# ayotoasset/AdditiveCausalExpansion

Measured on AMD Instinct MI355X. Metric: log-marg-lik+grad evals/sec at n=16384,d=20; Cholesky GF/s vs MFMA peak, higher is better.
Workload: dtype f64; 1 GPU; C2: n=16384, d=20, Matern32, ns basis B=10, fp64; one para_update (kernel assembly + SPD inverse/log-det + all P gradients + RMSE/evidence + Nadam step) per step; n=16384, p=20, B=10, kernel=Matern32, parallelism=single

## Files before the change

additivecausalexpansion_amd/__init__.py:

```python
from ._lib import AceError, Context, default_context, lib
from .native import (
    DMat, Adam_cpp, Nadam_cpp, Nesterov_cpp, coef_contract, grad_Matern_cpp, grad_SE_cpp,
    invkernel_cpp, kernmat_Matern32_cpp, kernmat_Matern32_symmetric_cpp, kernmat_SE_cpp,
    kernmat_SE_symmetric_cpp, mu_solution_cpp, ncs_basis, ncs_basis_deriv, norm_clip_cpp,
    normalize_test, normalize_train, pred_cpp, pred_marginal_cpp, robust_levels, stats_cpp)
from .model import (
    DeviceModel, KernelClass_Matern32_R6, KernelClass_SE_R6, comm_unique_id, optAdam, optNadam,
    optNesterov, set_optimizer)
from .r6 import R6KernelMatern32, R6KernelSE
from .train import (
    AceFit, ace_train, coef_posterior, linear_spline, ns_spline, predict_ace, response_surface,
    robust_treatment, set_basis, set_initial_parameters, square_spline)
```

additivecausalexpansion_amd/_lib.py:

```python
from __future__ import annotations

import ctypes
import os
import threading

import numpy as np

_HERE = os.path.dirname(os.path.abspath(__file__))
LIB_PATH = os.environ.get("ACE_LIB_PATH") or os.path.join(_HERE, "libace_hip.so")

ACE_KERNEL_SE = 0
ACE_KERNEL_MATERN32 = 1
KIND = {"SE": ACE_KERNEL_SE, "Matern32": ACE_KERNEL_MATERN32}

_D = ctypes.POINTER(ctypes.c_double)
_I64 = ctypes.c_int64
_I32 = ctypes.POINTER(ctypes.c_int32)
_vp = ctypes.c_void_p

SIGNATURES = {
    "ace_abi_version": (ctypes.c_int, []),
    "ace_create": (ctypes.c_int, [ctypes.c_int, ctypes.POINTER(_vp)]),
    "ace_destroy": (None, [_vp]),
    "ace_last_error": (ctypes.c_char_p, [_vp]),
# ... 35 lines not shown
                                    _vp, _vp, ctypes.c_double, ctypes.c_double, _D, _D, _D]),
    "ace_pred_marginal_dev": (ctypes.c_int, [_vp, _I64, _I64, _D, _D, ctypes.c_double,
                                             ctypes.c_double, _vp, _vp, _vp, ctypes.c_double,
                                             ctypes.c_double, ctypes.c_double, ctypes.c_int, _D,
                                             _D, _D, _D]),
    "ace_nesterov": (ctypes.c_int, [_I64, ctypes.c_double, ctypes.c_double, _D, _D, _D]),
    "ace_nadam": (ctypes.c_int, [_I64, ctypes.c_double, ctypes.c_double, ctypes.c_double,
                                 ctypes.c_double, ctypes.c_double, _D, _D, _D, _D]),
    "ace_adam": (ctypes.c_int, [_I64, ctypes.c_double, ctypes.c_double, ctypes.c_double,
                                ctypes.c_double, ctypes.c_double, _D, _D, _D, _D]),
    "ace_norm_clip": (None, [ctypes.c_int, _I64, _D, ctypes.c_double]),
    "ace_ncs_basis": (ctypes.c_int, [_I64, _D, _I64, _D, _D, ctypes.POINTER(_I64)]),
    "ace_ncs_basis_deriv": (ctypes.c_int, [_I64, _D, _I64, _D, _D, ctypes.POINTER(_I64)]),
    "ace_normalize_train": (ctypes.c_int, [_I64, ctypes.c_int, ctypes.c_int, _D, _D, _D, _D]),
    "ace_normalize_test": (ctypes.c_int, [_I64, ctypes.c_int, ctypes.c_int, _D, _D, _D, _I64]),
    "ace_model_create": (ctypes.c_int, [_vp, ctypes.c_int, _I64, ctypes.c_int, ctypes.c_int,
                                        ctypes.POINTER(_vp)]),
    "ace_model_destroy": (None, [_vp]),
    "ace_model_set_data": (ctypes.c_int, [_vp, _D, _D, _D, ctypes.c_double]),
    "ace_model_para_update": (ctypes.c_int, [_vp, ctypes.c_int, _D, _D, _D, _D]),
    "ace_model_train_stats": (ctypes.c_int, [_vp, _D, _D]),
    "ace_model_get_inverse": (ctypes.c_int, [_vp, _D]),
    "ace_model_apply_inverse": (ctypes.c_int, [_vp, _I64, _D, _D]),
    "ace_model_predict": (ctypes.c_int, [_vp, _D, _I64, _D, _D, ctypes.c_double, ctypes.c_double,
                                         _D, _D, _D]),
    "ace_model_predict_marginal": (ctypes.c_int, [_vp, _D, _I64, _D, _D, _D, ctypes.c_double,
                                                  ctypes.c_double, ctypes.c_int, _D, _D, _D,
                                                  _D]),
    "ace_model_predict_marginal_groups": (ctypes.c_int, [_vp, _D, _I64, _D, _D, ctypes.c_double,
                                                         ctypes.c_double, ctypes.c_int, _I32, _D,
# ... 134 lines not shown
```

additivecausalexpansion_amd/csrc/ace_api.cpp:

```cpp
#include <hip/hip_runtime.h>
#include <hip/hip_ext.h>

#include <algorithm>
#include <chrono>
#include <cmath>
#include <cstdio>
#include <cstring>
#include <limits>
#include <string>
#include <thread>
#include <vector>

#include "../../include/ace_hip.h"

#include "ace_common.h"
#include "ace_internal.h"
#include "ace_model.h"

using namespace ace;

std::string g_create_err;

namespace {
double sync_timeout_s() {
// ... 484 lines not shown
    const int per = asm_fill_on() ? assembly_persist_per_cu(s.kind, s.PM, s.B) : 0;
    if (per > 0) {
      fill = AsmFill{s.kind, s.PM, s.B, s.ZS, 32 * R * per, ps, w.npad, w.naug, tv, sig, w.A.d(), w.aq.i()};
      sy.fill = asm_fill;
      sy.fill_arg = &fill;
    }
  } else {
    ck(ctx, launch_assembly(0, s.kind, s.PM, ps, ps, w.npad, s.B, s.ZS, tv, sig, w.A.d(), w.naug,
                            nullptr, st, nullptr, 0, 1, 2),
       "assembly");
  }
  if (ev_asm) ck(ctx, hipEventRecord(ev_asm[1], st), "event");
  ck(ctx, run_sweep(w.bufs(), st, &sy, tmg), "sweep");
}

void build_grad_tiles(ace_ctx *ctx, int64_t n, DBuf &tiles, int64_t *ntiles, int64_t *ndiag) {
  *ntiles = grad_ntiles(n);
  *ndiag = -1;
  const int S = grad_order_block();
  if (S <= 0) return;
  const int64_t ntr = (n + AT - 1) / AT;
  std::vector<Tile> lst, low;
  for (int64_t I = 0; I < ntr; ++I) lst.push_back(Tile{(int)I, (int)I});
  for (int64_t I = 1; I < ntr; ++I)
    for (int64_t J = 0; J < I; ++J) low.push_back(Tile{(int)I, (int)J});
  const std::vector<Tile> o = xcd_update_order(low, S);
  lst.insert(lst.end(), o.begin(), o.end());
  alloc(ctx, tiles, lst.size() * sizeof(Tile), "alloc grad tiles");
  upload_bytes(ctx, tiles.p, lst.data(), lst.size() * sizeof(Tile), "upload grad tiles");
  *ntiles = (int64_t)lst.size();
  *ndiag = ntr;
}

static bool slice_norms_on() {
  static const bool v = env_int("ACE_NORMS", 1) != 0;
  return v;
}

namespace {

void model_pipeline(ace_model *m, SweepWork &w, const double *theta, int use_mu, bool timed,
// ... 2 lines not shown
  hipStream_t st = ctx->stream;
  const Shape &s = m->s;
  TabView tv = tab_view(m->tab, s);
  double sig = 0.0;
  if (theta_dev) {
    ck(ctx, launch_make_tab(theta_dev, s.B, s.p, s.PM, m->tab.d(), st), "tables");
    tv.sig = m->tab.d() + 2 * s.B * s.PM + s.B;
  } else {
    std::vector<double> tab = make_tab(theta, s);
    double *h = m->hio.ensure(ctx, tab.size() + m->res.bytes / sizeof(double));
    std::copy(tab.begin(), tab.end(), h);
    ck(ctx, hipMemcpyAsync(m->tab.p, h, tab.size() * sizeof(double), hipMemcpyHostToDevice, st),
       "upload tables");
    sig = std::exp(theta[0]);
  }
  const PairSide ps = m->side.view(m->n);
  if (m->norms.p) {
    const int NS = s.kind == ACE_KERNEL_MATERN32 ? s.B + 1 : s.B;
    ck(ctx, launch_slice_norms(ps.X, s.PM, m->npad, s.B, NS, tv.wk,
                               s.kind == ACE_KERNEL_MATERN32 ? tv.wg + (s.B - 1) * s.PM : tv.wk,
                               m->norms.d(), st),
       "slice norms");
    tv.norms = m->norms.d();
    tv.ldn = m->npad;
  }
  const int ts = m->tset;
  SweepTiming tmg;
  const size_t nset = m->ev_upd.size() / 2;
  tmg.ev = m->ev_upd.data() + ts * nset;
  tmg.nev = (int)nset;
  tmg.used = &m->upd_used[ts];
// ... 207 lines not shown
}

int ace_model_set_data(ace_model *m, const double *y, const double *X, const double *Z,
                       double std_y) {
  if (!m) return ACE_ERR_ARG;
  ace_ctx *ctx = m->ctx;
  ACE_TRY
  ck(ctx, hipSetDevice(ctx->device), "hipSetDevice");
  arg(ctx, y && (m->s.p == 0 || X) && (m->s.B == 1 || Z), "null argument");
  if (m->shard) {
    shard_set_data(m->shard, y, X, Z);
    m->std_y = std_y;
    m->has_data = true;
    return ACE_OK;
  }
  upload_side(ctx, m->side, m->s, X, Z, m->n, m->npad);
  std::vector<double> yp((size_t)m->npad, 0.0);
  std::copy(y, y + m->n, yp.begin());
  upload_bytes(ctx, m->y.p, yp.data(), yp.size() * sizeof(double), "upload y");
  m->std_y = std_y;
  sync(ctx);
  m->has_data = true;
  return ACE_OK;
  ACE_CATCH
}

#ifdef ACE_HOST_TRACE
static double host_us() {
  return std::chrono::duration<double, std::micro>(std::chrono::steady_clock::now().time_since_epoch())
      .count();
}
static double g_ht_exit = 0.0;
#define ACE_HT(name) const double name = host_us()
// ... 100 lines not shown

int ace_model_get_inverse(ace_model *m, double *inv) {
  if (!m) return ACE_ERR_ARG;
  ace_ctx *ctx = m->ctx;
  ACE_TRY
  ck(ctx, hipSetDevice(ctx->device), "hipSetDevice");
  arg(ctx, inv != nullptr, "null argument");
  if (m->shard) {
    shard_get_inverse(m->shard, inv);
    return ACE_OK;
  }
  DBuf out;
  alloc(ctx, out, (size_t)(m->n * m->n) * sizeof(double), "alloc inverse");
  ck(ctx, launch_sym_from_lower(m->sw.A.d(), m->naug, m->n, -1.0, out.d(), m->n, ctx->stream),
     "symmetrize");
  download(ctx, inv, out.d(), (size_t)(m->n * m->n), "download inverse");
  sync(ctx);
  return ACE_OK;
  ACE_CATCH
}

int ace_model_profile(ace_model *m, int enable) {
  if (!m) return ACE_ERR_ARG;
  m->prof = enable != 0;
  m->pend = -1;
  for (int j = 0; j < 6; ++j) {
    m->t_ms[j] = 0;
    m->t_launch[j] = 0;
    m->t_work[j] = 0;
  }
  return ACE_OK;
}
// ... 153 lines not shown
```

additivecausalexpansion_amd/csrc/ace_host.cpp:

```cpp
#include <algorithm>
#include <cmath>
#include <vector>

#include "../../include/ace_hip.h"

namespace {

bool all_finite(int64_t P, const double *g) {
  for (int64_t j = 0; j < P; ++j)
    if (!std::isfinite(g[j])) return false;
  return true;
}

}

extern "C" {

int ace_nesterov(int64_t P, double learn_rate, double momentum, double *nu, const double *grad,
                 double *para) {
  const bool ok = all_finite(P, grad);
  for (int64_t j = 0; j < P; ++j) {
    nu[j] = momentum * nu[j] + learn_rate * grad[j];
    para[j] = para[j] + nu[j];
  }
// ... 203 lines not shown
    const double p = std::min(t * by, 1.0);
    const double index = 1 + (double)(nx - 1) * p;
    const double lo = std::floor(index), hi = std::ceil(index);
    double q = x[(size_t)lo - 1];
    const double xh = x[(size_t)hi - 1];
    if (index > lo && xh != q) {
      const double h = index - lo;
      q = (1 - h) * q + h * xh;
    }
    thresholds[t] = q;
  }
  for (int64_t i = 0; i < nx; ++i) {
    int t = 0;
    while (t < n_steps && !(var[i] <= thresholds[t])) ++t;
    level[i] = t;
  }
  return ACE_OK;
}

int ace_coef_contract(int64_t nx, int B, int64_t nz, const double *mean, const double *cov,
                      const double *W, double offset, double scale, double shift, double noise,
                      double *map, double *ci, double *var) {
  if (nx < 1 || nz < 1 || B < 1 || !mean || !cov || !W || !map || !ci || !var) return ACE_ERR_ARG;
  const int64_t N = nx * nz;
  std::vector<double> wj((size_t)B);
  for (int64_t j = 0; j < nz; ++j) {
    for (int b = 0; b < B; ++b) wj[(size_t)b] = W[j + nz * b];
    for (int64_t c = 0; c < nx; ++c) {
      double a = 0.0, q = 0.0;
      for (int b = 0; b < B; ++b) a += wj[(size_t)b] * mean[c + nx * b];
// ... 19 lines not shown
```

additivecausalexpansion_amd/csrc/ace_internal.h:

```cpp
#pragma once
#include <functional>
#include <vector>
#include <hip/hip_runtime.h>
#include <stdint.h>
#include <stdlib.h>

namespace ace {

inline int env_int(const char *name, int dflt) {
  const char *e = getenv(name);
  return e ? atoi(e) : dflt;
}
inline bool env_set(const char *name) { return getenv(name) != nullptr; }

#ifndef ACE_NB
#define ACE_NB 256
#endif
constexpr int NB = ACE_NB;
constexpr int SUB = 64;
constexpr int UT = 128;
constexpr int AUG = 128;
constexpr int AT = 64;
constexpr int PMAX = 64;
constexpr int BMAX = 32;
// ... 10 lines not shown
  int I, J;
};

struct TabView {
  const double *wk, *wg, *lam;
  const double *sig = nullptr;
  const double *norms = nullptr;
  int64_t ldn = 0;
};

struct PairSide {
  const double *X;
  const double *Z;
  const double *LZ;
  int64_t n;
};

hipError_t launch_assembly(int mode, int kind, int PM, PairSide rows,
                           PairSide cols, int64_t npad, int B, int ZS,
                           TabView tab, double sig, double *out, int64_t ld,
                           double *cube, hipStream_t st, const Tile *tiles = nullptr,
                           int64_t ntiles = 0, int G = 1, int part = 0, int b0 = 0,
                           int b1 = -1);
hipError_t launch_kdiag(int kind, PairSide S, int ZS, TabView tab, int b0, int b1, double *out,
                        hipStream_t st);

hipError_t launch_assembly_mm(int kind, int PM, PairSide S, int64_t npad, int B, int ZS,
                              TabView tab, double sig, double *out, int64_t ld,
                              double *kcopy, hipStream_t st, const Tile *tiles,
                              int64_t ntiles, int G, int part = 0);
hipError_t launch_assembly_persist(int kind, int PM, PairSide S, int64_t npad, int B, int ZS,
// ... 224 lines not shown
```

additivecausalexpansion_amd/csrc/ace_model.h:

```cpp
#pragma once
#include <functional>

#include "ace_common.h"
#include "ace_internal.h"

struct SweepWork {
  DBuf A, Ps[8], Ws[8], SW, S0, S1, piv, flag, order, xtiles, ptiles, gorder, htiles;
  int Z = 2;
  DBuf gtiles;
  DBuf aq;
  DBuf bq;
  int breserve = 0;
  DBuf gpart, gwork, gsum;
  DBuf norms;
  int64_t ngtiles = 0, ngdiag = -2;
  std::vector<int64_t> xoff, poff, hoff;
  int64_t glen = 0;
  std::vector<hipEvent_t> ev;
  int64_t n = 0, npad = 0, naug = 0, norder = 0;
  SweepWork() = default;
  SweepWork(const SweepWork &) = delete;
  ~SweepWork() {
    for (auto &e : ev) (void)hipEventDestroy(e);
  }
// ... 122 lines not shown
                             m ? tv.wg + (s.B - 1) * s.PM : tv.wk, buf.d(), st),
     "slice norms");
  tv.norms = buf.d();
  tv.ldn = np;
  return tv;
}

struct ace_model {
  ace_ctx *ctx = nullptr;
  Shape s{};
  int64_t n = 0, npad = 0, naug = 0, ntiles = 0, ntr = 0;
  double std_y = 1.0;
  bool has_data = false;
  bool has_inverse = false;
  SideBufs side;
  DBuf y, tab, alpha, gpart, gwork;
  DBuf res;
  DView gsum, sums, scal;
  DBuf norms;
  DBuf gtiles;
  int64_t ngdiag = -1;
  PinnedBuf hio;
  SweepWork sw;
  SweepWork sw2;
  bool prof = false;
  hipEvent_t ev_asm[4] = {}, ev_grad[4] = {};
  std::vector<hipEvent_t> ev_upd;
  std::vector<double> upd_flops;
  int upd_used[2] = {0, 0};
  int tset = 0, pend = -1;
  double t_ms[6] = {0, 0, 0, 0, 0, 0};
  int64_t t_launch[6] = {0, 0, 0, 0, 0, 0};
  double t_work[6] = {0, 0, 0, 0, 0, 0};
  ShardModel *shard = nullptr;
};


void assemble_and_sweep(ace_ctx *ctx, SweepWork &w, const Shape &s, const PairSide &ps,
                        const TabView &tv, double sig, const double *y, int64_t n,
                        const SweepTiming *tmg, hipEvent_t *ev_asm);
void build_grad_tiles(ace_ctx *ctx, int64_t n, DBuf &tiles, int64_t *ntiles, int64_t *ndiag);

struct PredOps {
  ace_ctx *ctx = nullptr;
  int64_t n = 0;
  const double *w = nullptr;
  std::function<void(const double *V, int64_t ldv, int64_t k, double *out, DBuf &tmp)> symm;
  std::function<void(const double *V, int64_t ldv, int64_t k, double *out)> trmm;
  std::function<void(const double *V, int64_t ldv, int64_t k, double *out, DBuf &tmp)> symv;
  const double *sdiag = nullptr;
  std::function<void(double *dst)> ainv_w;
  std::function<void(double *buf, int64_t count)> allreduce;
  std::function<const double *(int64_t c0, int64_t nc, int64_t *ld, DBuf &scratch)> cross;
  std::function<void(double *dst)> kdiag;
  std::function<const double *(int64_t *ld, DBuf &scratch)> kxx;
};
// ... 4 lines not shown
```

additivecausalexpansion_amd/csrc/ace_pairs.hip:

```cpp
#include <algorithm>
#include <cstdlib>

#include "ace_internal.h"

namespace ace {

#define SQRT3 1.7320508075688772

__device__ __forceinline__ double sgn(double x) {
  return (double)((0.0 < x) - (x < 0.0));
}

template <int KIND, bool CROSS>
__device__ __forceinline__ double kval(int b, double r2, double lam, double zlo,
                                       double zhi, double lzlo, double lzhi) {
  if (KIND == 0) {
    if (b == 0) return exp(lam - r2);
    if (zlo == 0.0 || zhi == 0.0) return 0.0;
    return (sgn(zlo) * sgn(zhi)) * exp(((lam - r2) + lzlo) + lzhi);
  } else {
    const double t = sqrt(r2);
    const double e = (1.0 + SQRT3 * t) * exp(lam - SQRT3 * t);
    if (b == 0) return e;
    if (zlo == 0.0) return 0.0;
// ... 555 lines not shown
    else ACE_ASM(1, 2);
  }
#undef ACE_ASM
  return hipGetLastError();
}

bool pairs_use_mm(int PM, bool grad) {
  static const int v = [] {
    const char *e = getenv("ACE_PAIRS");
    return !e ? 2 : (e[0] == 'm' ? 1 : (e[0] == 'v' ? 0 : 2));
  }();
  (void)grad;
  return v != 0;
}

hipError_t launch_assembly(int mode, int kind, int PM, PairSide R, PairSide C, int64_t npad,
                           int B, int ZS, TabView tab, double sig, double *out, int64_t ld,
                           double *cube, hipStream_t st, const Tile *tiles, int64_t ntiles,
                           int G, int part, int b0, int b1) {
  if (b1 < 0) b1 = B;
  if (mode == 0 && pairs_use_mm(PM, false) && mm_lds_ok(PM, B, kind, false))
    return launch_assembly_mm(kind, PM, R, npad, B, ZS, tab, sig, out, ld, cube, st, tiles,
                              ntiles, G, part);
  if (mode == 2 && !cube && !tiles && pairs_use_mm(PM, false) && cross_mm_lds_ok(PM, B, kind))
    return launch_cross_mm(kind, PM, R, C, B, ZS, tab, b0, b1, out, ld, st);
  if (part == 2) return hipSuccess;
  switch (PM) {
#define ACE_CASE(P) \
  case P:           \
    return asm_pm<P>(mode, kind, R, C, npad, B, ZS, tab, sig, out, ld, cube, st, tiles, ntiles, G, \
// ... 62 lines not shown
```

additivecausalexpansion_amd/csrc/ace_pairs_mm.hip:

```cpp
#include <map>
#include <mutex>
#include <tuple>
#include <type_traits>

#include "ace_internal.h"
#include "ace_wgtime.h"

namespace ace {

typedef double d4 __attribute__((ext_vector_type(4)));

#ifndef ACE_MM_PG
#define ACE_MM_PG 2
#endif
#ifndef ACE_MM_GRAD_WPE
#define ACE_MM_GRAD_WPE 4
#endif
#ifndef ACE_MM_QG
#define ACE_MM_QG 4
#endif
#ifndef ACE_MM_QG2
#define ACE_MM_QG2 1
#endif
#ifndef ACE_GRAD_TAIL4
#define ACE_GRAD_TAIL4 1
#endif
#define MM_PAIR_FENCE(cb, v) \
  if (ACE_MM_PG > 0 && ((4 * (cb) + (v) + 1) % (ACE_MM_PG > 0 ? ACE_MM_PG : 1)) == 0) \
    __builtin_amdgcn_sched_barrier(0)

#define SQRT3 1.7320508075688772

__device__ __forceinline__ double sel_f64(bool c, double a, double b) {
  const unsigned long long ua = __double_as_longlong(a), ub = __double_as_longlong(b);
  const unsigned lo = c ? (unsigned)ua : (unsigned)ub;
  const unsigned hi = c ? (unsigned)(ua >> 32) : (unsigned)(ub >> 32);
  return __longlong_as_double((long long)(((unsigned long long)hi << 32) | lo));
}

__device__ __forceinline__ double sgn_mm(double x) {
// ... 233 lines not shown
}

__device__ __forceinline__ void tile_of(const Tile *tiles, int64_t t, int64_t &I, int64_t &J) {
  if (tiles) {
    const Tile tt = tiles[t];
    I = tt.I;
    J = tt.J;
  } else {
    I = (int64_t)((sqrt(8.0 * (double)t + 1.0) - 1.0) * 0.5);
    while ((I + 1) * (I + 2) / 2 <= t) ++I;
    while (I * (I + 1) / 2 > t) --I;
    J = t - I * (I + 1) / 2;
  }
}

__host__ __device__ constexpr int xj_pitch(int PM) { return PM + 1; }

struct MmLayout {
  int etab, xj, xi, z, lz, nc, nr, w, red, red_slices, total;
};

__host__ __device__ inline MmLayout mm_layout(int PM, int B, int KIND, bool grad, int nwave = 4) {
  MmLayout o;
  const int NS = (grad && KIND == 1) ? B + 1 : B;
  int off = 0;
  o.etab = off;
  off += (grad && ACE_GRAD_EXP == 2) ? 128 : (!grad && ACE_ASM_EXP == 2) ? 64 : 32;
  o.xj = off;
  off += 64 * xj_pitch(PM);
  o.xi = off;
// ... 203 lines not shown
  const int lr = lane & 15, lk = lane >> 4;
  const int wr = w & 3, cbase = 16 * CB * (w >> 2);
  const int64_t R0 = I * AT, C0 = J * AT, n = S.n;
  const int rl = 16 * wr + lr;
  const int64_t r = R0 + rl;
  constexpr int XP = xj_pitch(PM);
  const MmLds L = mm_stage<PM, KIND, false, ASM_NT>(lds, S, B, ZS, tab.wk, tab.wk, R0, C0, tid,
                                                    tab.norms, tab.ldn);
  RowX<PM> xr;
  xr.load(S.X + r * PM, lk);
  double kf[CB][4];
#pragma unroll
  for (int cb = 0; cb < CB; ++cb)
#pragma unroll
    for (int v = 0; v < 4; ++v) kf[cb][v] = 0.0;
  auto slices = [&](auto diag) {
    constexpr bool DG = decltype(diag)::value;
    for (int b = 0; b < B; ++b) {
      double zr = 1.0, lzr = 0.0;
      if (b > 0) {
        zr = S.Z[r * ZS + b - 1];
        if (KIND == 0) lzr = S.LZ[r * ZS + b - 1];
      }
      d4 acc[CB];
      gemm1_mm<XP, CB>(L.XJ, xr, L.W + b * PM, lr, lk, acc, cbase);
      const double sr = L.Nr[b * 64 + rl];
      const double *nc = L.Nc + b * 64 + cbase;
      const double lam = tab.lam[b];
  #pragma unroll
      for (int cb = 0; cb < CB; ++cb)
  #pragma unroll
        for (int v = 0; v < 4; ++v) {
          const int cl = 16 * cb + lk + 4 * v;
// ... 259 lines not shown
  int64_t I, J;
  if (tiles) {
    I = tiles[t].I;
    J = tiles[t].J;
    if (I < 0) {
      for (int64_t e = threadIdx.x; e < ldg; e += NT) gpart[t * ldg + e] = 0.0;
      return;
    }
  } else if (DG) {
    I = J = blockIdx.x;
  } else {
    tile_of(nullptr, blockIdx.x, I, J);
    ++I;
  }
  if (G > 1) A += (lcol(J * AT, G) - J * AT) * ld;
  const int tid = threadIdx.x, lane = tid & 63, w = tid >> 6;
  const int lr = lane & 15, lk = lane >> 4;
  const int wr = w & 3;
  const int cbase = 16 * CB * (w >> 2);
  const int64_t R0 = I * AT, C0 = J * AT, n = S.n;
  const int rl = 16 * wr + lr;
  const int64_t r = R0 + rl;
  const bool rvalid = r < n;
  const double *wlast = (KIND == 1) ? tab.wg + (B - 1) * PM : tab.wk;
  double av[CB][4], alc[CB][4];
#pragma unroll
  for (int cb = 0; cb < CB; ++cb)
#pragma unroll
    for (int v = 0; v < 4; ++v) {
      const int64_t c = C0 + cbase + 16 * cb + lk + 4 * v;
// ... 22 lines not shown
    }
  RowX<PM, XIL> xr;
  xr.load(XIL ? L.XI + rl * (PM + 1) : S.X + r * PM, lk);
  const int i4 = lane >> 4, m4 = (lane >> 2) & 3, j4 = lane & 3;
  double x4[NT4 > 0 ? NT4 : 1];
  if (TAIL4) {
    const int rr = 16 * wr + 4 * m4 + i4;
#pragma unroll
    for (int t4 = 0; t4 < NT4; ++t4) {
      const int nn = 16 * NQF + 4 * t4 + j4;
      x4[t4] = XIL ? L.XI[rr * (PM + 1) + nn] : (R0 + rr < n ? S.X[(R0 + rr) * PM + nn] : 0.0);
    }
  }
  double fc[CB][4];
  d4 acc[CB];
  if (KIND == 1) {
    gemm1_mm<XP, CB>(L.XJ, xr, L.W + B * PM, lr, lk, acc, cbase);
    const double sr = L.Nr[B * 64 + rl];
    const double *nc = L.Nc + B * 64 + cbase;
#pragma unroll
    for (int cb = 0; cb < CB; ++cb)
#pragma unroll
      for (int v = 0; v < 4; ++v) {
        const int cl = 16 * cb + lk + 4 * v;
        double rt2 = fmax(fma(-2.0, acc[cb][v], sr + nc[cl]), 0.0);
        if (DG && C0 + cbase + cl == r) rt2 = 0.0;
        fc[cb][v] = 1.0 + sqrt_pk(3.0 * rt2);
      }
  }
  auto finish = [&](int b, const double *red, int i, bool summed = false) {
    double g = 0.0;
    if (i < PM) {
#pragma unroll
      for (int q = 0; q < NWV; ++q) g += red[q * RS + i];
      const double *cc = red + NWV * RS;
      double gc = 0.0;
      if (summed) {
        for (int c = 0; c < 64; ++c) {
          const double x = L.XJ[c * XP + i];
          gc = fma(x * x, cc[c], gc);
        }
      } else {
        for (int c = 0; c < 64; ++c) {
          const double x = L.XJ[c * XP + i];
          gc = fma(x * x, (cc[c] + cc[64 + c]) + (cc[128 + c] + cc[192 + c]), gc);
        }
      }
      g += gc;
    } else {
#pragma unroll
      for (int q = 0; q < NWV; ++q) g += red[q * RS + PM];
    }
    gpart[t * ldg + (int64_t)b * NV + i] = g;
  };
  constexpr bool per_slice = PS;
#ifndef ACE_DIAG_GRAD
#define ACE_DIAG_GRAD 0
#endif
  const int bstop = (ACE_DIAG_GRAD & 3) == 1 ? B : (ACE_DIAG_GRAD & 3) == 2 ? B - 1 : 0;
#pragma unroll 1
  for (int b = B - 1; b >= bstop; --b) {
    double *red = L.Red + (per_slice ? b : (b & 1)) * PER;
    double zr = 1.0, lzr = 0.0;
    if (b > 0) {
      zr = S.Z[r * ZS + b - 1];
      if (KIND == 0) lzr = S.LZ[r * ZS + b - 1];
    }
    __builtin_amdgcn_s_setprio(2);
    gemm1_mm<XP, CB>(L.XJ, xr, L.W + b * PM, lr, lk, acc, cbase);
    __builtin_amdgcn_s_setprio(0);
    const double sr = L.Nr[b * 64 + rl];
    const double *nc = L.Nc + b * 64 + cbase;
    const double *zcol = L.Z + (b - 1) * 64 + cbase;
    const double *lzcol = L.LZ + (b - 1) * 64 + cbase;
    const double lam = tab.lam[b];
    double gl = 0.0, rs = 0.0;
#pragma unroll
// ... 4 lines not shown
        const int64_t c = C0 + cbase + cl;
        constexpr double R2MIN = KIND == 1 ? 1e-300 : 0.0;
        double r2 = fmax(fma(-2.0, acc[cb][v], sr + nc[cl]), R2MIN);
        if (DG && c == r) r2 = R2MIN;
        const double zc = zcol[cl];
        const double lzc = KIND == 0 ? lzcol[cl] : 0.0;
        const bool rlo = DG && r < c;
        const double zlo = rlo ? zr : zc, zhi = rlo ? zc : zr;
        double kb, f = 1.0;
        if (KIND == 0) {
          const double kz = (sgn_mm(zlo) * sgn_mm(zhi)) *
                            exp_grad(((lam - r2) + (rlo ? lzr : lzc)) + (rlo ? lzc : lzr), L.E);
          kb = sel_f64(zlo == 0.0 || zhi == 0.0, 0.0, kz);
        } else {
          const double tt = (ACE_DIAG_GRAD & 4) ? r2 : sqrt_gs(r2);
          f = 1.0 + SQRT3 * tt;
          const double e = (ACE_DIAG_GRAD & 8) ? f * (lam - SQRT3 * tt) : f * exp_grad(lam - SQRT3 * tt, L.E);
          kb = (e * zlo) * zhi;
        }
        const double tk = tv[cb][v] * kb;
        gl += tk;
        double u;
        if (KIND == 0) {
          u = tk;
        } else {
          u = (ACE_DIAG_GRAD & 16) ? tk * fc[cb][v] : tk * rcp_nr_mm(fc[cb][v]);
          fc[cb][v] = f;
        }
        acc[cb][v] = u;
        rs += u;
        MM_PAIR_FENCE(cb, v);
// ... 102 lines not shown
      if (tid <= PM) finish(b, red, tid);
    }
  }
  ACE_WGT_MARK(1);
  tr += xor_row(tr, 1);
  tr += xor_row(tr, 2);
  tr += xor_row(tr, 4);
  tr += xor_row(tr, 8);
  tr = add_xor16(tr);
  tr = add_xor32(tr);
  double *str = L.Red + L.red_slices * PER;
  if (lane == 0) str[w] = tr;
  __syncthreads();
  if (per_slice && !(ACE_DIAG_GRAD & 64)) {
    for (int e = tid; e < B * 64; e += NT) {
      double *cc = L.Red + (e >> 6) * PER + NWV * RS;
      const int c = e & 63;
      cc[c] = (cc[c] + cc[64 + c]) + (cc[128 + c] + cc[192 + c]);
    }
    __syncthreads();
    for (int e = tid; e < B * NV; e += NT) {
      const int bb = e / NV, i = e - bb * NV;
      finish(bb, L.Red + bb * PER, i, true);
    }
  }
  if (tid == 0) {
    double s = 0.0;
#pragma unroll
    for (int q = 0; q < NWV; ++q) s += str[q];
    gpart[t * ldg + (int64_t)B * NV] = s;
  }
}

#ifndef ACE_MM_GRAD_CB
#define ACE_MM_GRAD_CB 2
#endif
__host__ __device__ constexpr int grad_cb(int PM, int kind) {
// ... 649 lines not shown
```

additivecausalexpansion_amd/csrc/ace_predict.cpp:

```cpp
#include <hip/hip_runtime.h>

#include <algorithm>
#include <cstdlib>
#include <cmath>
#include <functional>
#include <vector>

#include "../../include/ace_hip.h"

#include "ace_common.h"
#include "ace_internal.h"
#include "ace_model.h"

using namespace ace;

namespace {

constexpr int64_t NXC = 8192;

struct PredScratch {
  DBuf K, T, Kxx;
};

void symm_resident(ace_model *m, const double *V, int64_t ldv, bool vt, int64_t k, double *out,
// ... 340 lines not shown
  upload_side(ctx, test, s, X2, ones.data(), nx, nx);
  const PairSide train = m->shard ? shard_train_side(m->shard) : m->side.view(n);
  const int64_t chunk = std::min<int64_t>(coef_chunk(B), nx);
  alloc(ctx, dK, (size_t)(chunk * B * n) * sizeof(double), "alloc Kc");
  std::vector<double> h((size_t)(chunk * B * n));
  for (int64_t c0 = 0; c0 < nx; c0 += chunk) {
    const int64_t nc = std::min<int64_t>(chunk, nx - c0), ldk = nc * B;
    PairSide tc = test.view(nc);
    tc.X += c0 * s.PM;
    tc.Z += c0 * s.ZS;
    tc.LZ += c0 * s.ZS;
    slice_assembly(ctx, s, tc, train, tv, dK.d());
    download(ctx, h.data(), dK.d(), (size_t)(ldk * n), "download Kc");
    sync(ctx);
    for (int b = 0; b < B; ++b)
      for (int64_t q = 0; q < n; ++q)
        for (int64_t c = 0; c < nc; ++c)
          out[c0 + c + nx * (q + n * b)] = h[(size_t)(c + nc * b + q * ldk)];
  }
}

void coef_once(ace_model *m, const double *theta, int64_t nx, const double *X2, double *mean,
               double *P) {
  ace_ctx *ctx = m->ctx;
  hipStream_t st = ctx->stream;
  const Shape &s = m->s;
  const int64_t n = m->n;
  const int B = s.B;
  const double mu = theta[1];
  std::vector<double> tab = make_tab(theta, s, false);
  DBuf dtab, dw, dsv, ddiag, dscal, dtmp, dpart, dres;
  upload(ctx, dtab, tab.data(), tab.size(), "upload tables");
  const TabView tv = tab_view(dtab, s);
// ... 97 lines not shown
}

}

extern "C" {

int ace_model_apply_inverse(ace_model *m, int64_t k, const double *V, double *out) {
  if (!m) return ACE_ERR_ARG;
  ace_ctx *ctx = m->ctx;
  ACE_TRY
  ck(ctx, hipSetDevice(ctx->device), "hipSetDevice");
  arg(ctx, k >= 1 && V && out, "bad shape / null argument");
  require_inverse(m);
  const int64_t n = m->n;
  DBuf dV, dout, dtmp;
  upload(ctx, dV, V, (size_t)(n * k), "upload V");
  alloc(ctx, dout, (size_t)(n * k) * sizeof(double), "alloc out");
  symm_resident(m, dV.d(), n, false, k, dout.d(), dtmp);
  if (m->shard) shard_allreduce_sum(m->shard, dout.d(), n * k);
  download(ctx, out, dout.d(), (size_t)(n * k), "download out");
  sync(ctx);
  return ACE_OK;
  ACE_CATCH
}

int ace_model_predict(ace_model *m, const double *theta, int64_t nx, const double *X2,
                      const double *Z2, double mean_y, double std_y, double *map, double *ci,
                      double *var) {
  if (!m) return ACE_ERR_ARG;
  ace_ctx *ctx = m->ctx;
  ACE_TRY
  ck(ctx, hipSetDevice(ctx->device), "hipSetDevice");
  arg(ctx, nx >= 1 && theta && map && ci && var && (m->s.p == 0 || X2) && (m->s.B == 1 || Z2),
      "bad shape / null argument");
  require_inverse(m);
  predict_impl(m, theta, nx, X2, Z2, false, nullptr, 0, mean_y, std_y, 1.0, map, ci, var, nullptr);
// ... 168 lines not shown
```

additivecausalexpansion_amd/native.py:

```python
from __future__ import annotations

import ctypes

import numpy as np

from ._lib import KIND, AceError, check, default_context, fmat, lib, ptr


def _ctx(ctx):
    return (ctx or default_context()).handle


class DMat:

    def __init__(self, handle, ctx):
        self.handle, self.ctx = handle, ctx
        r, c, sl = ctypes.c_int64(), ctypes.c_int64(), ctypes.c_int64()
        check(lib().ace_dmat_dims(handle, ctypes.byref(r), ctypes.byref(c), ctypes.byref(sl)))
        self.shape = (r.value, c.value) if sl.value == 1 else (r.value, c.value, sl.value)

    @classmethod
    def upload(cls, a, ctx=None):
        a = np.asarray(a, dtype=np.float64)
        dims = a.shape + (1,) * (3 - a.ndim)
# ... 336 lines not shown
    Z = _inplace(Z, "Z")
    mom = fmat(moments)
    check(lib().ace_normalize_test(X.shape[0], X.shape[1], Z.shape[1], ptr(X), ptr(Z), ptr(mom),
                                   mom.shape[0]))


def robust_levels(var, n_steps):
    v = np.ascontiguousarray(np.ravel(var), dtype=np.float64)
    thr = np.empty(max(int(n_steps), 0) + 1)
    level = np.empty(v.size, dtype=np.int32)
    check(lib().ace_robust_levels(v.size, ptr(v), int(n_steps), ptr(thr),
                                  level.ctypes.data_as(ctypes.POINTER(ctypes.c_int32))))
    return thr, level


def coef_contract(mean, cov, W, offset=0.0, scale=1.0, shift=0.0, noise=0.0):
    mf = fmat(mean)
    if mf.ndim != 2:
        raise AceError("mean must be nx x B")
    nx, B = mf.shape
    cf = np.asfortranarray(np.asarray(cov, dtype=np.float64).reshape((nx, B, B), order="F"))
    Wf = np.asfortranarray(np.asarray(W, dtype=np.float64).reshape((-1, B), order="F"))
    nz = Wf.shape[0]
    mp = np.empty((nx, nz), order="F")
    var = np.empty((nx, nz), order="F")
    ci = np.empty((nx, nz, 2), order="F")
    check(lib().ace_coef_contract(nx, B, nz, ptr(mf), cf.ctypes.data_as(ctypes.POINTER(ctypes.c_double)),
                                  ptr(Wf), float(offset), float(scale), float(shift), float(noise),
                                  ptr(mp), ci.ctypes.data_as(ctypes.POINTER(ctypes.c_double)),
                                  ptr(var)))
# ... 2 lines not shown
```

include/ace_hip.h:

```cpp
#ifndef ACE_HIP_H
#define ACE_HIP_H

#include <stdint.h>

#ifdef __cplusplus
extern "C" {
#endif

#define ACE_ABI_VERSION 1

enum ace_kernel_kind { ACE_KERNEL_SE = 0, ACE_KERNEL_MATERN32 = 1 };

enum ace_status {
  ACE_OK = 0,
  ACE_ERR_ARG = 1,
  ACE_ERR_HIP = 2,
  ACE_ERR_OOM = 3,
  ACE_ERR_UNSUPPORTED = 4,
  ACE_ERR_NONFINITE = 5,
  ACE_ERR_INTERRUPTED = 6,
  ACE_ERR_TIMEOUT = 7
};

typedef struct ace_ctx ace_ctx;
// ... 84 lines not shown
int ace_adam(int64_t P, double iter, double learn_rate, double beta1,
             double beta2, double eps, double *m, double *v,
             const double *grad, double *para);

void ace_norm_clip(int flag, int64_t P, double *grads, double max_length);

int ace_ncs_basis(int64_t n, const double *x, int64_t nknots,
                  const double *knots, double *design, int64_t *ncols);
int ace_ncs_basis_deriv(int64_t n, const double *x, int64_t nknots,
                        const double *knots, double *design, int64_t *ncols);

int ace_normalize_train(int64_t n, int px, int pz, double *y, double *X,
                        double *Z, double *moments);
int ace_normalize_test(int64_t n, int px, int pz, double *X, double *Z,
                       const double *moments, int64_t moment_rows);

int ace_model_create(ace_ctx *ctx, int kind, int64_t n, int p, int B,
                     ace_model **out);
void ace_model_destroy(ace_model *m);
int ace_model_set_data(ace_model *m, const double *y, const double *X,
                       const double *Z, double std_y);
int ace_model_para_update(ace_model *m, int iter, double *theta, double *grad,
                          double *stats, double *mu_post);
int ace_model_train_stats(ace_model *m, const double *theta, double *stats);
int ace_model_get_inverse(ace_model *m, double *inv);
int ace_model_apply_inverse(ace_model *m, int64_t k, const double *V, double *out);

int ace_model_predict(ace_model *m, const double *theta, int64_t nx, const double *X2,
                      const double *Z2, double mean_y, double std_y, double *map, double *ci,
                      double *var);
// ... 69 lines not shown
```

Baseline: 13.61 evals/s.

## Reorder training rows by Z zero pattern and skip inactive basis slices per tile

When the data is loaded, rows are sorted by the nonzero pattern of the spline basis Z, and a per-64-row block bitmask of active slices is uploaded to the device. Assembly and gradient kernels read the mask per tile pair and skip slices that are identically zero, and the gradient tile order is weighted by active-slice count. The permutation is undone on the host for inverse downloads, apply_inverse and the Kc output. This aims to remove wasted work on zero basis columns. It adds host-side sorting and permutation copies, extra branches in the kernels, and depends on Z being sparse, which natural-spline bases over sorted data may or may not be.

```diff
diff --git a/additivecausalexpansion_amd/__init__.py b/additivecausalexpansion_amd/__init__.py
--- a/additivecausalexpansion_amd/__init__.py
+++ b/additivecausalexpansion_amd/__init__.py
@@ -3,7 +3,8 @@
     DMat, Adam_cpp, Nadam_cpp, Nesterov_cpp, coef_contract, grad_Matern_cpp, grad_SE_cpp,
     invkernel_cpp, kernmat_Matern32_cpp, kernmat_Matern32_symmetric_cpp, kernmat_SE_cpp,
     kernmat_SE_symmetric_cpp, mu_solution_cpp, ncs_basis, ncs_basis_deriv, norm_clip_cpp,
-    normalize_test, normalize_train, pred_cpp, pred_marginal_cpp, robust_levels, stats_cpp)
+    normalize_test, normalize_train, pred_cpp, pred_marginal_cpp, robust_levels, stats_cpp,
+    zero_pattern_order)
 from .model import (
     DeviceModel, KernelClass_Matern32_R6, KernelClass_SE_R6, comm_unique_id, optAdam, optNadam,
     optNesterov, set_optimizer)
diff --git a/additivecausalexpansion_amd/_lib.py b/additivecausalexpansion_amd/_lib.py
--- a/additivecausalexpansion_amd/_lib.py
+++ b/additivecausalexpansion_amd/_lib.py
@@ -73,6 +73,8 @@
     "ace_ncs_basis_deriv": (ctypes.c_int, [_I64, _D, _I64, _D, _D, ctypes.POINTER(_I64)]),
     "ace_normalize_train": (ctypes.c_int, [_I64, ctypes.c_int, ctypes.c_int, _D, _D, _D, _D]),
     "ace_normalize_test": (ctypes.c_int, [_I64, ctypes.c_int, ctypes.c_int, _D, _D, _D, _I64]),
+    "ace_zero_pattern_order": (ctypes.c_int, [_I64, ctypes.c_int, _D, ctypes.POINTER(_I64),
+                                              ctypes.POINTER(ctypes.c_uint32), _I32]),
     "ace_model_create": (ctypes.c_int, [_vp, ctypes.c_int, _I64, ctypes.c_int, ctypes.c_int,
                                         ctypes.POINTER(_vp)]),
     "ace_model_destroy": (None, [_vp]),
diff --git a/additivecausalexpansion_amd/csrc/ace_api.cpp b/additivecausalexpansion_amd/csrc/ace_api.cpp
--- a/additivecausalexpansion_amd/csrc/ace_api.cpp
+++ b/additivecausalexpansion_amd/csrc/ace_api.cpp
@@ -522,7 +522,8 @@
   ck(ctx, run_sweep(w.bufs(), st, &sy, tmg), "sweep");
 }
 
-void build_grad_tiles(ace_ctx *ctx, int64_t n, DBuf &tiles, int64_t *ntiles, int64_t *ndiag) {
+void build_grad_tiles(ace_ctx *ctx, int64_t n, DBuf &tiles, int64_t *ntiles, int64_t *ndiag,
+                      const uint32_t *mask) {
   *ntiles = grad_ntiles(n);
   *ndiag = -1;
   const int S = grad_order_block();
@@ -532,7 +533,10 @@
   for (int64_t I = 0; I < ntr; ++I) lst.push_back(Tile{(int)I, (int)I});
   for (int64_t I = 1; I < ntr; ++I)
     for (int64_t J = 0; J < I; ++J) low.push_back(Tile{(int)I, (int)J});
-  const std::vector<Tile> o = xcd_update_order(low, S);
+  std::function<double(const Tile &)> cost;
+  if (mask)
+    cost = [mask](const Tile &t) { return 1.0 + __builtin_popcount(mask[t.I] & mask[t.J]); };
+  const std::vector<Tile> o = xcd_update_order(low, S, cost);
   lst.insert(lst.end(), o.begin(), o.end());
   alloc(ctx, tiles, lst.size() * sizeof(Tile), "alloc grad tiles");
   upload_bytes(ctx, tiles.p, lst.data(), lst.size() * sizeof(Tile), "upload grad tiles");
@@ -565,7 +569,7 @@
        "upload tables");
     sig = std::exp(theta[0]);
   }
-  const PairSide ps = m->side.view(m->n);
+  const PairSide ps = m->train_side();
   if (m->norms.p) {
     const int NS = s.kind == ACE_KERNEL_MATERN32 ? s.B + 1 : s.B;
     ck(ctx, launch_slice_norms(ps.X, s.PM, m->npad, s.B, NS, tv.wk,
@@ -803,9 +807,56 @@
     m->has_data = true;
     return ACE_OK;
   }
+  const Shape &s = m->s;
+  const int64_t n = m->n;
+  const int zs = s.B - 1, mode = zskip_mode(n);
+  m->perm.clear();
+  m->has_zmask = false;
+  std::vector<double> Xp, Zp, yp((size_t)m->npad, 0.0);
+  std::copy(y, y + n, yp.begin());
+  if (mode > 0 && zs >= 1 && zs <= 32 && pairs_use_mm(s.PM, false) &&
+      mm_lds_ok(s.PM, s.B, s.kind, false) && mm_lds_ok(s.PM, s.B, s.kind, true)) {
+    const uint32_t all = zs >= 32 ? 0xffffffffu : ((uint32_t)1 << zs) - 1;
+    std::vector<uint32_t> bm((size_t)(m->npad / AT), all);
+    std::vector<int64_t> perm((size_t)n);
+    int32_t has = 0;
+    arg(ctx, ace_zero_pattern_order(n, zs, Z, perm.data(), bm.data(), &has) == ACE_OK,
+        "zero-pattern order");
+    bool ident = true;
+    for (int64_t k = 0; k < n && ident; ++k) ident = perm[(size_t)k] == k;
+    if (mode == 2 && !ident) {
+      Xp.resize((size_t)(n * s.p));
+      Zp.resize((size_t)(n * zs));
+      for (int i = 0; i < s.p; ++i)
+        for (int64_t k = 0; k < n; ++k) Xp[(size_t)(k + i * n)] = X[perm[(size_t)k] + i * n];
+      for (int b = 0; b < zs; ++b)
+        for (int64_t k = 0; k < n; ++k) Zp[(size_t)(k + b * n)] = Z[perm[(size_t)k] + b * n];
+      for (int64_t k = 0; k < n; ++k) yp[(size_t)k] = y[perm[(size_t)k]];
+      X = Xp.data();
+      Z = Zp.data();
+      m->perm = perm;
+    } else if (!ident) {
+      for (int64_t k = 0; k < n / AT; ++k) {
+        uint32_t w = 0;
+        for (int b = 0; b < zs; ++b)
+          for (int64_t j = AT * k; j < AT * (k + 1); ++j)
+            if (Z[j + b * n] != 0.0) w |= (uint32_t)1 << b;
+        bm[(size_t)k] = w;
+      }
+    }
+    bool any = false;
+    for (uint32_t w : bm) any = any || w != all;
+    if (any) {
+      alloc(ctx, m->zmask, bm.size() * sizeof(uint32_t), "alloc slice masks");
+      upload_bytes(ctx, m->zmask.p, bm.data(), bm.size() * sizeof(uint32_t), "upload slice masks");
+      m->has_zmask = true;
+    }
+    int64_t nt = 0;
+    build_grad_tiles(ctx, n, m->gtiles, &nt, &m->ngdiag,
+                     (any && !m->perm.empty()) ? bm.data() : nullptr);
+    arg(ctx, nt == m->ntiles, "gradient tile list changed size");
+  }
   upload_side(ctx, m->side, m->s, X, Z, m->n, m->npad);
-  std::vector<double> yp((size_t)m->npad, 0.0);
-  std::copy(y, y + m->n, yp.begin());
   upload_bytes(ctx, m->y.p, yp.data(), yp.size() * sizeof(double), "upload y");
   m->std_y = std_y;
   sync(ctx);
@@ -936,8 +987,19 @@
   alloc(ctx, out, (size_t)(m->n * m->n) * sizeof(double), "alloc inverse");
   ck(ctx, launch_sym_from_lower(m->sw.A.d(), m->naug, m->n, -1.0, out.d(), m->n, ctx->stream),
      "symmetrize");
-  download(ctx, inv, out.d(), (size_t)(m->n * m->n), "download inverse");
+  if (m->perm.empty()) {
+    download(ctx, inv, out.d(), (size_t)(m->n * m->n), "download inverse");
+    sync(ctx);
+    return ACE_OK;
+  }
+  const int64_t n = m->n;
+  std::vector<double> h((size_t)(n * n));
+  download(ctx, h.data(), out.d(), h.size(), "download inverse");
   sync(ctx);
+  for (int64_t j = 0; j < n; ++j) {
+    double *col = inv + m->perm[(size_t)j] * n;
+    for (int64_t i = 0; i < n; ++i) col[m->perm[(size_t)i]] = h[(size_t)(i + j * n)];
+  }
   return ACE_OK;
   ACE_CATCH
 }
diff --git a/additivecausalexpansion_amd/csrc/ace_host.cpp b/additivecausalexpansion_amd/csrc/ace_host.cpp
--- a/additivecausalexpansion_amd/csrc/ace_host.cpp
+++ b/additivecausalexpansion_amd/csrc/ace_host.cpp
@@ -241,6 +241,41 @@
     int t = 0;
     while (t < n_steps && !(var[i] <= thresholds[t])) ++t;
     level[i] = t;
+  }
+  return ACE_OK;
+}
+
+int ace_zero_pattern_order(int64_t n, int ZS, const double *Z, int64_t *perm, uint32_t *blockmask,
+                           int32_t *has_mask) {
+  if (n < 1 || ZS < 0 || (ZS > 0 && !Z) || !perm) return ACE_ERR_ARG;
+  const int W = (ZS + 63) / 64 > 0 ? (ZS + 63) / 64 : 1;
+  std::vector<uint64_t> pat((size_t)n * W, 0);
+  std::vector<int> cnt((size_t)n, 0);
+  for (int b = 0; b < ZS; ++b)
+    for (int64_t r = 0; r < n; ++r)
+      if (Z[r + (int64_t)b * n] != 0.0) {
+        pat[(size_t)r * W + b / 64] |= (uint64_t)1 << (b % 64);
+        ++cnt[(size_t)r];
+      }
+  for (int64_t r = 0; r < n; ++r) perm[r] = r;
+  std::stable_sort(perm, perm + n, [&](int64_t a, int64_t c) {
+    if (cnt[(size_t)a] != cnt[(size_t)c]) return cnt[(size_t)a] < cnt[(size_t)c];
+    for (int w = W - 1; w >= 0; --w)
+      if (pat[(size_t)a * W + w] != pat[(size_t)c * W + w])
+        return pat[(size_t)a * W + w] < pat[(size_t)c * W + w];
+    return false;
+  });
+  const bool mask = ZS <= 32 && blockmask != nullptr;
+  if (has_mask) *has_mask = mask ? 1 : 0;
+  if (!mask) return ACE_OK;
+  const uint32_t all = ZS >= 32 ? 0xffffffffu : ((uint32_t)1 << ZS) - 1;
+  const int64_t nblk = (n + 63) / 64;
+  for (int64_t k = 0; k < nblk; ++k) {
+    uint32_t m = 0;
+    if (64 * (k + 1) > n) m = all;
+    else
+      for (int64_t j = 64 * k; j < 64 * (k + 1); ++j) m |= (uint32_t)pat[(size_t)perm[j] * W];
+    blockmask[k] = m;
   }
   return ACE_OK;
 }
diff --git a/additivecausalexpansion_amd/csrc/ace_internal.h b/additivecausalexpansion_amd/csrc/ace_internal.h
--- a/additivecausalexpansion_amd/csrc/ace_internal.h
+++ b/additivecausalexpansion_amd/csrc/ace_internal.h
@@ -48,7 +48,10 @@
   const double *Z;
   const double *LZ;
   int64_t n;
-};
+  const uint32_t *mask = nullptr;
+};
+
+int zskip_mode(int64_t n);
 
 hipError_t launch_assembly(int mode, int kind, int PM, PairSide rows,
                            PairSide cols, int64_t npad, int B, int ZS,
diff --git a/additivecausalexpansion_amd/csrc/ace_model.h b/additivecausalexpansion_amd/csrc/ace_model.h
--- a/additivecausalexpansion_amd/csrc/ace_model.h
+++ b/additivecausalexpansion_amd/csrc/ace_model.h
@@ -160,6 +160,14 @@
   bool has_data = false;
   bool has_inverse = false;
   SideBufs side;
+  std::vector<int64_t> perm;
+  DBuf zmask;
+  bool has_zmask = false;
+  PairSide train_side() const {
+    PairSide ps = side.view(n);
+    if (has_zmask) ps.mask = static_cast<const uint32_t *>(zmask.p);
+    return ps;
+  }
   DBuf y, tab, alpha, gpart, gwork;
   DBuf res;
   DView gsum, sums, scal;
@@ -185,7 +193,8 @@
 void assemble_and_sweep(ace_ctx *ctx, SweepWork &w, const Shape &s, const PairSide &ps,
                         const TabView &tv, double sig, const double *y, int64_t n,
                         const SweepTiming *tmg, hipEvent_t *ev_asm);
-void build_grad_tiles(ace_ctx *ctx, int64_t n, DBuf &tiles, int64_t *ntiles, int64_t *ndiag);
+void build_grad_tiles(ace_ctx *ctx, int64_t n, DBuf &tiles, int64_t *ntiles, int64_t *ndiag,
+                      const uint32_t *mask = nullptr);
 
 struct PredOps {
   ace_ctx *ctx = nullptr;
diff --git a/additivecausalexpansion_amd/csrc/ace_pairs.hip b/additivecausalexpansion_amd/csrc/ace_pairs.hip
--- a/additivecausalexpansion_amd/csrc/ace_pairs.hip
+++ b/additivecausalexpansion_amd/csrc/ace_pairs.hip
@@ -593,6 +593,11 @@
   return v != 0;
 }
 
+int zskip_mode(int64_t n) {
+  static const int v = env_set("ACE_ZSKIP") ? std::max(0, std::min(2, env_int("ACE_ZSKIP", 2))) : -1;
+  return v >= 0 ? v : (n > 8192 ? 2 : 1);
+}
+
 hipError_t launch_assembly(int mode, int kind, int PM, PairSide R, PairSide C, int64_t npad,
                            int B, int ZS, TabView tab, double sig, double *out, int64_t ld,
                            double *cube, hipStream_t st, const Tile *tiles, int64_t ntiles,
diff --git a/additivecausalexpansion_amd/csrc/ace_pairs_mm.hip b/additivecausalexpansion_amd/csrc/ace_pairs_mm.hip
--- a/additivecausalexpansion_amd/csrc/ace_pairs_mm.hip
+++ b/additivecausalexpansion_amd/csrc/ace_pairs_mm.hip
@@ -24,6 +24,9 @@
 #endif
 #ifndef ACE_GRAD_TAIL4
 #define ACE_GRAD_TAIL4 1
+#endif
+#ifndef ACE_DIAG_GRAD
+#define ACE_DIAG_GRAD 0
 #endif
 #define MM_PAIR_FENCE(cb, v) \
   if (ACE_MM_PG > 0 && ((4 * (cb) + (v) + 1) % (ACE_MM_PG > 0 ? ACE_MM_PG : 1)) == 0) \
@@ -287,6 +290,15 @@
   }
 }
 
+__device__ __forceinline__ unsigned tile_slices(const uint32_t *__restrict__ mask, int64_t I,
+                                                int64_t J) {
+  if (!mask) return ~0u;
+  return (unsigned)__builtin_amdgcn_readfirstlane((int)(mask[I] & mask[J]));
+}
+__device__ __forceinline__ bool slice_on(unsigned act, int b) {
+  return b == 0 || ((act >> (b - 1)) & 1u) != 0;
+}
+
 __host__ __device__ constexpr int xj_pitch(int PM) { return PM + 1; }
 
 struct MmLayout {
@@ -520,9 +532,11 @@
   for (int cb = 0; cb < CB; ++cb)
 #pragma unroll
     for (int v = 0; v < 4; ++v) kf[cb][v] = 0.0;
+  const unsigned act = tile_slices(S.mask, I, J);
   auto slices = [&](auto diag) {
     constexpr bool DG = decltype(diag)::value;
     for (int b = 0; b < B; ++b) {
+      if (!slice_on(act, b)) continue;
       double zr = 1.0, lzr = 0.0;
       if (b > 0) {
         zr = S.Z[r * ZS + b - 1];
@@ -812,6 +826,7 @@
     ++I;
   }
   if (G > 1) A += (lcol(J * AT, G) - J * AT) * ld;
+  const unsigned act0 = tile_slices(S.mask, I, J);
   const int tid = threadIdx.x, lane = tid & 63, w = tid >> 6;
   const int lr = lane & 15, lk = lane >> 4;
   const int wr = w & 3;
@@ -864,19 +879,41 @@
   }
   double fc[CB][4];
   d4 acc[CB];
+  unsigned act = act0;
   if (KIND == 1) {
-    gemm1_mm<XP, CB>(L.XJ, xr, L.W + B * PM, lr, lk, acc, cbase);
-    const double sr = L.Nr[B * 64 + rl];
-    const double *nc = L.Nc + B * 64 + cbase;
-#pragma unroll
-    for (int cb = 0; cb < CB; ++cb)
-#pragma unroll
-      for (int v = 0; v < 4; ++v) {
-        const int cl = 16 * cb + lk + 4 * v;
-        double rt2 = fmax(fma(-2.0, acc[cb][v], sr + nc[cl]), 0.0);
-        if (DG && C0 + cbase + cl == r) rt2 = 0.0;
-        fc[cb][v] = 1.0 + sqrt_pk(3.0 * rt2);
-      }
+    int top = B - 1;
+    if (S.mask) {
+      const unsigned m = act0 & (B - 1 >= 32 ? ~0u : (1u << (B - 1)) - 1u);
+      top = m ? 32 - __builtin_clz(m) : 0;
+      const unsigned below = top >= 32 ? ~0u : (1u << top) - 1u;
+      act = m | (((m << 1) | 1u) & below);
+    }
+    const int s = top == B - 1 ? B : top + 1;
+    gemm1_mm<XP, CB>(L.XJ, xr, L.W + s * PM, lr, lk, acc, cbase);
+    const double sr = L.Nr[s * 64 + rl];
+    const double *nc = L.Nc + s * 64 + cbase;
+    if (top == B - 1) {
+#pragma unroll
+      for (int cb = 0; cb < CB; ++cb)
+#pragma unroll
+        for (int v = 0; v < 4; ++v) {
+          const int cl = 16 * cb + lk + 4 * v;
+          double rt2 = fmax(fma(-2.0, acc[cb][v], sr + nc[cl]), 0.0);
+          if (DG && C0 + cbase + cl == r) rt2 = 0.0;
+          fc[cb][v] = 1.0 + sqrt_pk(3.0 * rt2);
+        }
+    } else {
+#pragma unroll
+      for (int cb = 0; cb < CB; ++cb)
+#pragma unroll
+        for (int v = 0; v < 4; ++v) {
+          const int cl = 16 * cb + lk + 4 * v;
+          double r2 = fmax(fma(-2.0, acc[cb][v], sr + nc[cl]), 1e-300);
+          if (DG && C0 + cbase + cl == r) r2 = 1e-300;
+          const double tt = (ACE_DIAG_GRAD & 4) ? r2 : sqrt_gs(r2);
+          fc[cb][v] = fma(SQRT3, tt, 1.0);
+        }
+    }
   }
   auto finish = [&](int b, const double *red, int i, bool summed = false) {
     double g = 0.0;
@@ -904,13 +941,16 @@
     gpart[t * ldg + (int64_t)b * NV + i] = g;
   };
   constexpr bool per_slice = PS;
-#ifndef ACE_DIAG_GRAD
-#define ACE_DIAG_GRAD 0
-#endif
   const int bstop = (ACE_DIAG_GRAD & 3) == 1 ? B : (ACE_DIAG_GRAD & 3) == 2 ? B - 1 : 0;
+  int nrun = 0;
 #pragma unroll 1
   for (int b = B - 1; b >= bstop; --b) {
-    double *red = L.Red + (per_slice ? b : (b & 1)) * PER;
+    if (!slice_on(act, b)) {
+      if (tid < NV) gpart[t * ldg + (int64_t)b * NV + tid] = 0.0;
+      continue;
+    }
+    double *red = L.Red + (per_slice ? b : (nrun & 1)) * PER;
+    ++nrun;
     double zr = 1.0, lzr = 0.0;
     if (b > 0) {
       zr = S.Z[r * ZS + b - 1];
@@ -945,7 +985,7 @@
           kb = sel_f64(zlo == 0.0 || zhi == 0.0, 0.0, kz);
         } else {
           const double tt = (ACE_DIAG_GRAD & 4) ? r2 : sqrt_gs(r2);
-          f = 1.0 + SQRT3 * tt;
+          f = fma(SQRT3, tt, 1.0);
           const double e = (ACE_DIAG_GRAD & 8) ? f * (lam - SQRT3 * tt) : f * exp_grad(lam - SQRT3 * tt, L.E);
           kb = (e * zlo) * zhi;
         }
@@ -1078,6 +1118,7 @@
   __syncthreads();
   if (per_slice && !(ACE_DIAG_GRAD & 64)) {
     for (int e = tid; e < B * 64; e += NT) {
+      if (!slice_on(act, e >> 6)) continue;
       double *cc = L.Red + (e >> 6) * PER + NWV * RS;
       const int c = e & 63;
       cc[c] = (cc[c] + cc[64 + c]) + (cc[128 + c] + cc[192 + c]);
@@ -1085,6 +1126,7 @@
     __syncthreads();
     for (int e = tid; e < B * NV; e += NT) {
       const int bb = e / NV, i = e - bb * NV;
+      if (!slice_on(act, bb)) continue;
       finish(bb, L.Red + bb * PER, i, true);
     }
   }
diff --git a/additivecausalexpansion_amd/csrc/ace_predict.cpp b/additivecausalexpansion_amd/csrc/ace_predict.cpp
--- a/additivecausalexpansion_amd/csrc/ace_predict.cpp
+++ b/additivecausalexpansion_amd/csrc/ace_predict.cpp
@@ -378,9 +378,11 @@
     download(ctx, h.data(), dK.d(), (size_t)(ldk * n), "download Kc");
     sync(ctx);
     for (int b = 0; b < B; ++b)
-      for (int64_t q = 0; q < n; ++q)
+      for (int64_t q = 0; q < n; ++q) {
+        const int64_t qo = m->perm.empty() ? q : m->perm[(size_t)q];
         for (int64_t c = 0; c < nc; ++c)
-          out[c0 + c + nx * (q + n * b)] = h[(size_t)(c + nc * b + q * ldk)];
+          out[c0 + c + nx * (qo + n * b)] = h[(size_t)(c + nc * b + q * ldk)];
+      }
   }
 }
 
@@ -508,12 +510,22 @@
   require_inverse(m);
   const int64_t n = m->n;
   DBuf dV, dout, dtmp;
-  upload(ctx, dV, V, (size_t)(n * k), "upload V");
+  const std::vector<int64_t> &perm = m->perm;
+  std::vector<double> hp;
+  if (!perm.empty()) {
+    hp.resize((size_t)(n * k));
+    for (int64_t c = 0; c < k; ++c)
+      for (int64_t q = 0; q < n; ++q) hp[(size_t)(q + c * n)] = V[perm[(size_t)q] + c * n];
+  }
+  upload(ctx, dV, perm.empty() ? V : hp.data(), (size_t)(n * k), "upload V");
   alloc(ctx, dout, (size_t)(n * k) * sizeof(double), "alloc out");
   symm_resident(m, dV.d(), n, false, k, dout.d(), dtmp);
   if (m->shard) shard_allreduce_sum(m->shard, dout.d(), n * k);
-  download(ctx, out, dout.d(), (size_t)(n * k), "download out");
+  download(ctx, perm.empty() ? out : hp.data(), dout.d(), (size_t)(n * k), "download out");
   sync(ctx);
+  if (!perm.empty())
+    for (int64_t c = 0; c < k; ++c)
+      for (int64_t q = 0; q < n; ++q) out[perm[(size_t)q] + c * n] = hp[(size_t)(q + c * n)];
   return ACE_OK;
   ACE_CATCH
 }
diff --git a/additivecausalexpansion_amd/native.py b/additivecausalexpansion_amd/native.py
--- a/additivecausalexpansion_amd/native.py
+++ b/additivecausalexpansion_amd/native.py
@@ -374,6 +374,21 @@
     return thr, level
 
 
+def zero_pattern_order(Z):
+    Zf = fmat(Z)
+    if Zf.ndim != 2 or Zf.shape[0] < 1:
+        raise AceError("Z must be n x ZS with n >= 1")
+    n, ZS = Zf.shape
+    perm = np.empty(n, dtype=np.int64)
+    mask = np.zeros((n + 63) // 64, dtype=np.uint32)
+    has = np.zeros(1, dtype=np.int32)
+    check(lib().ace_zero_pattern_order(n, ZS, ptr(Zf) if ZS else None,
+                                       perm.ctypes.data_as(ctypes.POINTER(ctypes.c_int64)),
+                                       mask.ctypes.data_as(ctypes.POINTER(ctypes.c_uint32)),
+                                       has.ctypes.data_as(ctypes.POINTER(ctypes.c_int32))))
+    return perm, (mask if has[0] else None)
+
+
 def coef_contract(mean, cov, W, offset=0.0, scale=1.0, shift=0.0, noise=0.0):
     mf = fmat(mean)
     if mf.ndim != 2:
diff --git a/include/ace_hip.h b/include/ace_hip.h
--- a/include/ace_hip.h
+++ b/include/ace_hip.h
@@ -122,6 +122,9 @@
                         double *Z, double *moments);
 int ace_normalize_test(int64_t n, int px, int pz, double *X, double *Z,
                        const double *moments, int64_t moment_rows);
+
+int ace_zero_pattern_order(int64_t n, int ZS, const double *Z, int64_t *perm,
+                           uint32_t *blockmask, int32_t *has_mask);
 
 int ace_model_create(ace_ctx *ctx, int kind, int64_t n, int p, int B,
                      ace_model **out);
```

Result: faster. 14.13 evals/s (median of 6 runs) (+3.8%).
